# lfilipozzi/PathPlanning

Hardware: AMD Instinct MI355X
Metric: hybrid_astar_plans_per_sec_1024x1024 (higher is better)
Workload: dtype f64

## Files before the change

__graft_entry__.py:

```python
import os
import subprocess
import sys

os.environ.setdefault("GPU_MAX_HW_QUEUES", "2")

ROOT = os.path.dirname(os.path.abspath(__file__))
if ROOT not in sys.path:
    sys.path.insert(0, ROOT)


def build():
    from pathplanning_amd import build as b
    lib = b.build(force=False)
    assert os.path.exists(lib), lib
    b.build_pyplanning()
    b.build_plugin_test()
    b.build_pipeline_footprint_test()
    b.build_pipeline_postprocess_test()
    b.build_pipeline_revalidate_test()
    b.build_pipeline_stamp_test()
    b.build_stamp_rule_test()
    b.build_ticket_table_test()
    b.build_row_test()
    subprocess.check_call(["make", "-C", os.path.join(ROOT, "oracle"), os.path.join(ROOT, "oracle", "libppo.so")])
    if os.path.isdir("/root/reference/planner/src"):
        subprocess.check_call(["make", "-C", os.path.join(ROOT, "oracle"), "ref"])
    subprocess.check_call([sys.executable, "-c", "import ctypes, sys; ctypes.CDLL(sys.argv[1])", lib])
    import pathplanning_amd
    print("built", lib)


def smoke():
    sys.path.insert(0, os.path.join(ROOT, "tests"))
    import numpy as np
    import pathplanning_amd as pa
    import torch
    assert torch.cuda.is_available(), "smoke() needs a GPU"
    import oracle_lib as O
    w = O.synthetic_world(256, 6, 3)
    ctx = pa.Context(0)
    ms = pa.OccupancyMapSet.from_bounds(ctx, w.lb, w.ub, 0.1)
    ms.upload_dist2(w.d2())
    ms.upload_occupancy(w.occ())
    ms.upload_path_cost(w.pathcost())
    val = pa.StateValidatorOccupancyMap(ms)
    rng = np.random.RandomState(0)
    poses = np.column_stack([rng.uniform(-13, 13, 4096), rng.uniform(-13, 13, 4096), rng.uniform(-3.1, 3.1, 4096)])
    got = val.is_state_valid(poses)
    want = w.is_state_valid(poses).astype(bool)
    assert np.array_equal(got, want), "check_states mismatch"
    planner = pa.HybridAStarBatch(val, max_batch=2, max_nodes=32768)
    planner.initialize()
    starts = [[-10.0, -10.0, 0.0], [9.0, -9.0, 1.0]]
    goals = [[10.0, 10.0, 0.0], [-9.0, 8.0, -2.0]]
    res = planner.search_batch(starts, goals, [7, 8])
    h = O.Hybrid(w, table=planner.nonholo_table())
    for q in range(2):
        r = h.search(starts[q], goals[q], 7 + q)
        assert res[q].status == r["status"], (res[q].status, r["status"])
        assert np.array_equal(planner.get_expanded_of(q), r["expanded"]), "expansion order mismatch"
        if r["status"] == 0:
            assert abs(res[q].cost - r["cost"]) < 1e-5
    sys.path.insert(0, os.path.join(ROOT, "tests"))
    from gpu_common import valid_random_poses
    n = 72
    big = pa.HybridAStarBatch(val, max_batch=n, max_nodes=32768, search_rows=16)
    big.initialize()
    bs, bg = valid_random_poses(rng, w, n), valid_random_poses(rng, w, n)
    seeds = np.arange(n, dtype=np.uint64) + 100
    bres = big.search_batch(bs, bg, seeds)
    for q in range(0, n, 6):
        r = h.search(bs[q], bg[q], int(seeds[q]))
        assert bres[q].status == r["status"] and bres[q].n_expanded == len(r["expanded"]), (q, bres[q].status, bres[q].n_expanded, r["status"], len(r["expanded"]))
        assert np.array_equal(big.get_expanded_of(q), r["expanded"]), "expansion order mismatch (rows kernel)"
    import time
# ... 35 lines not shown
```

pathplanning_amd/build.py:

```python
import os
import subprocess
import sys

HERE = os.path.dirname(os.path.abspath(__file__))
CSRC = os.path.join(HERE, "csrc")
LIB_DIR = os.path.join(HERE, "lib")
LIB = os.path.join(LIB_DIR, "libpphip.so")
SOURCES = ["pp_capi.hip", "pp_kernels_basic.hip", "pp_paths.hip", "pp_footprint.hip", "pp_gvd.hip", "pp_wavefront.hip", "pp_wavefront_tiles.hip", "pp_planner.hip", "pp_rrt.hip", "pp_grid_astar.hip"]
HEADERS = sorted(f for f in os.listdir(CSRC) if f.endswith(".hpp")) + [os.path.join("..", "..", "include", "pp_hip.h")]
FLAGS = ["--offload-arch=gfx950", "-O3", "-std=c++17", "-ffp-contract=off", "-fPIC", "-shared"]


def hipcc():
    for c in (os.environ.get("HIPCC"), "/opt/rocm/bin/hipcc", "hipcc"):
        if c and (os.path.isabs(c) and os.path.exists(c) or not os.path.isabs(c)):
            return c
    return "hipcc"


def stale():
    if not os.path.exists(LIB):
        return True
    t = os.path.getmtime(LIB)
    deps = [os.path.join(CSRC, s) for s in SOURCES + HEADERS]
# ... 48 lines not shown
    cmd = ["g++", "-O2", "-std=c++17", src, "-o", out, "-L" + LIB_DIR, "-lpphip", "-Wl,-rpath,$ORIGIN"]
    if verbose:
        print(" ".join(cmd), file=sys.stderr)
    subprocess.check_call(cmd)
    return out


def build_pipeline_postprocess_test(verbose=True):
    build()
    out = os.path.join(LIB_DIR, "test_pipeline_postprocess")
    src = os.path.join(HERE, "..", "tests", "cpp", "test_pipeline_postprocess.cpp")
    cmd = ["g++", "-O2", "-std=c++17", src, "-o", out, "-L" + LIB_DIR, "-lpphip", "-Wl,-rpath,$ORIGIN"]
    if verbose:
        print(" ".join(cmd), file=sys.stderr)
    subprocess.check_call(cmd)
    return out


def build_pipeline_revalidate_test(verbose=True):
    build()
    out = os.path.join(LIB_DIR, "test_pipeline_revalidate")
    src = os.path.join(HERE, "..", "tests", "cpp", "test_pipeline_revalidate.cpp")
    cmd = ["g++", "-O2", "-std=c++17", src, "-o", out, "-L" + LIB_DIR, "-lpphip", "-Wl,-rpath,$ORIGIN"]
    if verbose:
        print(" ".join(cmd), file=sys.stderr)
    subprocess.check_call(cmd)
    return out


def build_pipeline_stamp_test(verbose=True):
    build()
    out = os.path.join(LIB_DIR, "test_pipeline_stamp")
    src = os.path.join(HERE, "..", "tests", "cpp", "test_pipeline_stamp.cpp")
    cmd = ["g++", "-O2", "-std=c++17", src, "-o", out, "-L" + LIB_DIR, "-lpphip", "-Wl,-rpath,$ORIGIN"]
    if verbose:
        print(" ".join(cmd), file=sys.stderr)
    subprocess.check_call(cmd)
    return out


def build_stamp_rule_test(verbose=True):
    os.makedirs(LIB_DIR, exist_ok=True)
    out = os.path.join(LIB_DIR, "test_stamp_rule")
    src = os.path.join(HERE, "..", "tests", "cpp", "test_stamp_rule.cpp")
    if os.path.exists(out) and os.path.getmtime(out) > max(os.path.getmtime(src), os.path.getmtime(os.path.join(CSRC, "pp_stamp_rule.hpp"))):
        return out
    cmd = ["g++", "-std=c++17", "-g", "-O1", "-ffp-contract=off", "-fsanitize=address,undefined", "-fno-sanitize-recover=all", "-I", CSRC, src, "-o", out]
    if verbose:
        print(" ".join(cmd), file=sys.stderr)
    subprocess.check_call(cmd)
    return out


def build_ticket_table_test(verbose=True):
    os.makedirs(LIB_DIR, exist_ok=True)
    out = os.path.join(LIB_DIR, "test_ticket_table")
    src = os.path.join(HERE, "..", "tests", "cpp", "test_ticket_table.cpp")
    if os.path.exists(out) and os.path.getmtime(out) > max(os.path.getmtime(src), os.path.getmtime(os.path.join(CSRC, "pp_ticket_table.hpp"))):
        return out
    cmd = ["g++", "-std=c++17", "-g", "-fsanitize=address,undefined", "-fno-sanitize-recover=all", "-I", CSRC, src, "-o", out]
    if verbose:
        print(" ".join(cmd), file=sys.stderr)
    subprocess.check_call(cmd)
    return out


def build_row_test(verbose=True):
    out = os.path.join(LIB_DIR, "test_row_primitives")
    src = os.path.join(HERE, "..", "tests", "cpp", "test_row_primitives.hip")
    if os.path.exists(out) and os.path.getmtime(out) > max(os.path.getmtime(src), os.path.getmtime(os.path.join(CSRC, "pp_row_primitives.hpp"))):
        return out
    cmd = [hipcc(), "--offload-arch=gfx950", "-O2", "-I", CSRC, "-I", os.path.join(HERE, "..", "include"), src, "-o", out]
    if verbose:
        print(" ".join(cmd), file=sys.stderr)
    subprocess.check_call(cmd)
    return out


if __name__ == "__main__":
    build(force="--force" in sys.argv)
    print(LIB)
    print(build_pyplanning())
    print(build_plugin_test())
    print(build_pipeline_footprint_test())
    print(build_pipeline_postprocess_test())
    print(build_pipeline_revalidate_test())
    print(build_pipeline_stamp_test())
    print(build_stamp_rule_test())
    print(build_ticket_table_test())
    print(build_row_test())
```

pathplanning_amd/csrc/pp_planner.hip:

```cpp
#include "pp_search_device.hpp"
#include "pp_row_primitives.hpp"
#include "pp_stamp_rule.hpp"

#include <cmath>
#include <cstring>
#include <memory>
#include <string>
#include <utility>
#include <vector>

using namespace ppd;

namespace {

struct Node {
	double x, y, t;
	double pathCost, totalCost;
	double length;
	double h;
	double sinT, cosT;
	int32_t parent;
	uint32_t key;
	int16_t action;
	uint8_t dead;
	uint8_t pad0;
	float dist0;
	uint8_t pad[8];
};
static_assert(sizeof(Node) == 96, "Node layout");

struct PathRec {
	double x, y, t, length;
	int32_t action;
	int32_t node;
};
static_assert(sizeof(PathRec) == 40, "PathRec layout");

struct SuspendRec {
	int32_t q, slot;
	int32_t heapSize, nNodes, nExpanded, nRngDraws, nRsAttempts, nRsLog, mtIdx;
	uint32_t seq;
	long long stateChecks, pathChecks;
	long long bandLo;
	int32_t nOutside, pad;
};

struct RsLogEntry {
	int32_t node, word;
	double t, u, v;
};
constexpr int kRsLogCap = 64;

struct KeySpace {
	int x0, y0, t0;
// ... 424 lines not shown
		if (a.from != a.from || a.to != a.to) {
			set_error(what(i) + " has a NaN in its window");
			return PP_ERR_INVALID;
		}
	}
	return PP_OK;
}

Footprint stamp_discs(const pp_footprint* fp, const pp_map* own)
{
	if (fp)
		return fp->fp;
	Footprint f {};
	f.n = 1;
	f.r[0] = own->minSafeRadius;
	return f;
}

int stamp_prepare_target(pp_map* map)
{
	if (map->occ32)
		return PP_OK;
	const size_t n = map->cells();
	PP_HIP_TRY(map->occ32.ensure(n * 4));
	PP_HIP_TRY(hipMemsetAsync(map->occ32, 0xFF, n * 4, map->ctx->stream));
	PP_HIP_TRY(hipStreamSynchronize(map->ctx->stream));
	return PP_OK;
}

int stamp_finish_target(pp_map* map)
{
	map->journal.clear();
	map->journal.shrink_to_fit();
	map->journalLost = true;
	if (int rc = pph::refresh_occupancy_views(map, map->ctx->stream))
		return rc;
	PP_HIP_TRY(hipStreamSynchronize(map->ctx->stream));
	return PP_OK;
}

template <typename Rec>
void records_out(const std::vector<Rec>& host, Rec* out)
{
	if (out)
		std::copy(host.begin(), host.end(), out);
}

void free_planner(pp_planner* p)
{
	if (!p)
		return;
#if PP_ROWS_STATS
	{
		unsigned long long h[24] = {};
		if (hipMemcpyFromSymbol(h, HIP_SYMBOL(g_rowsStats), sizeof h) == hipSuccess) {
			fprintf(stderr, "[rows stats] wave iterations with 1/2/3/4 busy rows: %llu %llu %llu %llu\n", h[1], h[2], h[3], h[4]);
			static const char* const names[14] = { "take", "set-aside", "pop+refill", "node", "child validity", "march", "truncate+cost", "cell-node+staging", "insert", "write", "rs", "endpoint", "keymap+heuristics", "voronoi" };
			unsigned long long tot = 0, it = h[1] + h[2] + h[3] + h[4];
			for (int i = 0; i < 14; i++)
				tot += h[8 + i];
			for (int i = 0; i < 14; i++)
				fprintf(stderr, "[rows stats]   %-18s %5.1f %%  %8.0f clk / wave iteration\n", names[i], 100.0 * (double)h[8 + i] / (double)(tot ? tot : 1), (double)h[8 + i] / (double)(it ? it : 1));
		}
	}
#endif
	pp_map* map = p->map;
	pph::footprint_release(p->footprint);
	delete p;
	pph::map_release(map);
}

}

enum class PlannerUse { Batches, Pipeline, PipelineLogged };
static int create_planner(pp_map* map, const pp_hybrid_params* params, int32_t max_batch, int32_t max_nodes_per_query, int32_t search_rows, PlannerUse use, pp_planner** out);

extern "C" {

int pp_planner_create(pp_map* map, const pp_hybrid_params* params, int32_t max_batch, int32_t max_nodes_per_query, pp_planner** out)
{
	return pp_planner_create_ex(map, params, max_batch, max_nodes_per_query, 0, out);
}

int pp_planner_create_ex(pp_map* map, const pp_hybrid_params* params, int32_t max_batch, int32_t max_nodes_per_query, int32_t search_rows, pp_planner** out)
{
	return create_planner(map, params, max_batch, max_nodes_per_query, search_rows, PlannerUse::Batches, out);
}

static int create_planner(pp_map* map, const pp_hybrid_params* params, int32_t max_batch, int32_t max_nodes_per_query, int32_t search_rows, PlannerUse use, pp_planner** out)
{
	const bool forPipeline = use != PlannerUse::Batches;
	if (!map || !params || !out || max_batch < 1 || max_nodes_per_query < 16 || search_rows < 0) {
		set_error("invalid arguments");
		return PP_ERR_INVALID;
	}
	if (!map->dist || !map->occ8 || !map->pathcost) {
		set_error("map set incomplete: upload dist2, occupancy and path cost first");
		return PP_ERR_INVALID;
	}
	PP_HIP_TRY(hipSetDevice(map->ctx->device));
	auto* p = new pp_planner();
	p->map = map;
	__atomic_add_fetch(&map->refs, 1, __ATOMIC_RELAXED);
	p->params = *params;
	p->maxBatch = max_batch;
	p->maxNodes = max_nodes_per_query;

	const double wheelbase = params->wheelbase, rearToCenter = 0.0;
	const double deltaMax = std::atan(wheelbase / std::sqrt(std::pow(params->min_turning_radius, 2) - std::pow(rearToCenter, 2)));
	p->deltas.push_back(0.0);
	for (unsigned int i = 0; i < params->num_generated_motion / 2; i++) {
		double delta = (i + 1) / 2.0 * deltaMax;
		p->deltas.push_back(delta);
		p->deltas.push_back(-delta);
	}
// ... 893 lines not shown
```

pathplanning_amd/csrc/pp_planner_rows.hpp:

```cpp
#ifndef PP_ROWS_FOOTPRINT
#error "pp_planner_rows.hpp is the body of the rows kernels of pp_planner.hip, which defines PP_ROWS_FOOTPRINT before each include"
#endif

#ifndef PP_ROWS_PREAMBLE_DONE
#define PP_ROWS_PREAMBLE_DONE 1
#ifndef PP_ROWS_STATS
#define PP_ROWS_STATS 0
#endif
#if PP_ROWS_STATS
__device__ unsigned long long g_rowsStats[24];
#endif
#ifndef PP_ROWS_WAVES_PER_WG
#define PP_ROWS_WAVES_PER_WG 4
#endif
#if PP_ROWS_STATS
#undef PP_ROWS_WAVES_PER_WG
#define PP_ROWS_WAVES_PER_WG 1
#endif
#ifndef PP_ROWS_EAGER_REFILL
#define PP_ROWS_EAGER_REFILL 1
#endif

#ifndef PP_PIPE_POLL_EVERY
#define PP_PIPE_POLL_EVERY 8
#endif
constexpr int kPollEvery = PP_PIPE_POLL_EVERY;
#endif

#if PP_ROWS_FOOTPRINT
#define PP_ROWS_KERNEL k_hybrid_search_rows_footprint
#define PP_ROWS_FOOT_ARG Footprint foot,
#else
#define PP_ROWS_KERNEL k_hybrid_search_rows
#define PP_ROWS_FOOT_ARG
#endif
template <bool kPiped>
__global__ void __launch_bounds__(64 * PP_ROWS_WAVES_PER_WG, PP_SEARCH_WAVES_PER_SIMD) PP_ROWS_KERNEL(SearchArgs A, PP_ROWS_FOOT_ARG int nQueries, const double* __restrict__ starts,
	const double* __restrict__ goals, const uint64_t* __restrict__ seeds, const float* __restrict__ costFields, Node* __restrict__ nodesBase,
	HeapEntry* __restrict__ heapBase, uint32_t* __restrict__ keymapBase, uint32_t* __restrict__ expandedBase, RsLogEntry* __restrict__ rsLogBase,
	PathRec* __restrict__ pathBase, unsigned long long* __restrict__ mtBase, DevResult* __restrict__ results, int* __restrict__ nextQuery,
	SuspendRec* __restrict__ suspended, const int32_t* __restrict__ order, int suspendAfter, int* __restrict__ suspendedCount, int* __restrict__ spareCount,
	HeapEntry* __restrict__ bandBase, double bandInvW, uint8_t* __restrict__ bandMetaBase, PipeView pipe)
{
#if PP_SEARCH_SETPRIO
	__builtin_amdgcn_s_setprio(PP_ROWS_PRIO);
#endif
	constexpr int kW = kPiped ? 1 : PP_ROWS_WAVES_PER_WG;
	const int lane = threadIdx.x & 63;
	const int waveIdx = (int)blockIdx.x * kW + (int)(threadIdx.x >> 6);
	if (waveIdx >= A.rowsWaves)
		return;
	const int rl = lane & (kRowLanes - 1);
	const int sb = (lane >> 4) * kRowSlots;
	constexpr bool piped = kPiped;
	if (piped) {
		int owner = 0;
		if (lane == 0)
			owner = __hip_atomic_compare_exchange_strong(pipe.waveAlive + waveIdx, &owner, 1, __ATOMIC_RELAXED, __ATOMIC_RELAXED, __HIP_MEMORY_SCOPE_AGENT) ? 0 : 1;
		if (__builtin_amdgcn_readfirstlane(owner))
			return;
		__builtin_amdgcn_fence(__ATOMIC_ACQUIRE, "agent");
	}
	int idleIters = 0;
// ... 52 lines not shown
	long long laneStateChecks = 0, lanePathChecks = 0, rsStateChecks = 0, rsPathChecks = 0;

	auto flush_spills = [&]() {
		wave_lds_sync();
		bool toHeap = false;
		if (rl < nSpill) {
			const HeapEntry mine = spillBuf[rl];
			const long long B = band_of_key(mine.ckey, bandInvW);
			toHeap = true;
			if (B >= bandLo && B < bandLo + kBands) {
				const int sl = (int)(B & (kBands - 1)), sh = (sl & 3) * 8;
				const uint32_t old = atomicAdd(&bandCnt[sl >> 2], 1u << sh);
				const int pos = (int)((old >> sh) & 0xFFu);
				if (pos < kBandCap) {
					ROW_BANDS[sl * kBandCap + pos] = mine;
					toHeap = false;
				} else {
					atomicSub(&bandCnt[sl >> 2], 1u << sh);
				}
			}
		}
		uint32_t hm = row_bits(__ballot(toHeap), lane);
		if (__builtin_expect(hm != 0u, false)) {
			wave_vmem_sync();
			if (rl == 0) {
				int hs = heapSize;
				for (uint32_t mm = hm; mm; mm &= mm - 1)
					heap_push(ROW_HEAP, hs, spillBuf[__ffs((int)mm) - 1]);
			}
			for (; hm; hm &= hm - 1) {
				const HeapEntry e = spillBuf[__ffs((int)hm) - 1];
				if (heapSize == 0 || heap_before(e, heapTop))
					heapTop = e;
				heapSize++;
			}
		}
		nSpill = 0;
		wave_lds_sync();
		wave_vmem_sync();
	};
	auto spill = [&](const HeapEntry& e) {
		if (!bandLoSet) {
			bandLo = (band_of_key(e.ckey, bandInvW) - 64) & ~3ll;
			bandLoSet = true;
		}
		if (rl == 0)
			spillBuf[nSpill] = e;
		nSpill++;
		nOutside++;
		if (key_before(e.ckey, e.nseq, lowK, lowS)) {
			lowK = e.ckey;
			lowS = e.nseq;
		}
		if (nSpill == kRowLanes)
			flush_spills();
	};
	auto push_open = [&](const HeapEntry& e) {
		bool toFront = true;
		if (frontCount < kRowLanes)
			toFront = nOutside == 0 || key_before(e.ckey, e.nseq, lowK, lowS) ||
				(frontCount > 0 && key_before(e.ckey, e.nseq, row_read64(front.ckey, lane, frontCount - 1), row_read(front.nseq, lane, frontCount - 1)));
		if (toFront) {
			HeapEntry sp;
			if (front_insert_row(front, frontCount, e, rl, lane, sp))
				spill(sp);
		} else {
			spill(e);
		}
	};
	auto refill = [&]() {
		if (nSpill > 0)
			flush_spills();
		long long bAbs = 0x7FFFFFFFFFFFFFFFll;
		const int w0 = (int)(bandLo >> 2);
#pragma unroll 1
		for (int step = 0; step < kBands / 64; step++) {
			const uint32_t w = bandCnt[(w0 + step * kRowLanes + rl) & (kBands / 4 - 1)];
			const uint32_t hit = row_bits(__ballot(w != 0u), lane);
			if (hit) {
				const int fl = __ffs((int)hit) - 1;
				const uint32_t wf = row_read(w, lane, fl);
				bAbs = bandLo + 4ll * (step * kRowLanes + fl) + ((__ffs((int)wf) - 1) >> 3);
				break;
			}
		}
		long long loadedTop = bandLo - 1;
		if (bAbs != 0x7FFFFFFFFFFFFFFFll) {
			const int sl = (int)(bAbs & (kBands - 1)), sh = (sl & 3) * 8;
			const int n = (int)((bandCnt[sl >> 2] >> sh) & 0xFFu);
			HeapEntry e;
			e.ckey = ~0ull;
			e.nseq = ~0u;
			e.node = 0;
			if (rl < n)
				e = ROW_BANDS[sl * kBandCap + rl];
			row_sort_entries(e.ckey, e.nseq, e.node, rl);
			front.ckey = e.ckey;
			front.nseq = e.nseq;
			front.node = e.node;
			frontCount = n;
			nOutside -= n;
			wave_lds_sync();
			if (rl == 0)
				bandCnt[sl >> 2] &= ~(0xFFu << sh);
			wave_lds_sync();
			bandLo = bAbs & ~3ll;
			loadedTop = bAbs;
		}
		lowK = ~0ull;
		lowS = ~0u;
		while (__builtin_expect(heapSize > 0 && (frontCount == 0 || key_before(heapTop.ckey, heapTop.nseq, row_read64(front.ckey, lane, frontCount - 1), row_read(front.nseq, lane, frontCount - 1))), false)) {
			wave_vmem_sync();
			const HeapEntry he = heap_pop_row(ROW_HEAP, heapSize, rl, lane, heapTop);
			wave_vmem_sync();
			nOutside--;
			HeapEntry sp;
			if (front_insert_row(front, frontCount, he, rl, lane, sp))
				spill(sp);
		}
		if (heapSize > 0 && key_before(heapTop.ckey, heapTop.nseq, lowK, lowS)) {
			lowK = heapTop.ckey;
			lowS = heapTop.nseq;
		}
		{
			const unsigned long long bk = cost_key((double)(loadedTop + 1) / bandInvW);
			if (bk < lowK || (bk == lowK && 0u < lowS)) {
				lowK = bk;
				lowS = 0u;
			}
		}
		wave_lds_sync();
		for (int i = 0; i < nSpill; i++) {
			const HeapEntry e = spillBuf[i];
			if (key_before(e.ckey, e.nseq, lowK, lowS)) {
				lowK = e.ckey;
				lowS = e.nseq;
			}
		}
	};
	auto set_slot = [&](size_t sl_) {
		slot = (int)sl_;
		nodes = nodesBase + (size_t)slot * A.maxNodes;
		keymap = keymapBase + (size_t)slot * A.ks.size();
	};
	auto finish = [&](const int status, const int solutionNode, const double solutionCost) {
		const long long nStateChecks = row_sum_i64(laneStateChecks, lane) + rsStateChecks;
		const long long pathChecksPacked = row_sum_i64(lanePathChecks, lane) + rsPathChecks;
		const long long pathChecks = pathChecksPacked & kGuardMask;
		wave_vmem_sync();
		if (rl == 0) {
			DevResult r;
			r.r.n_lattice_boundary_hits = (int32_t)(pathChecksPacked >> kGuardShift);
			r.r.reserved = 0;
			r.r.status = status;
			r.r.n_expanded = nExpanded;
			r.r.n_nodes = nNodes;
			r.r.n_path = 0;
			if (status == 0)
				r.r.n_path = write_path(nodes, solutionNode, pathBase + (size_t)q * A.maxPath, A.maxPath, piped ? pipe.pathHost + (size_t)q * (size_t)(3 * pipe.pathHostCap) : nullptr,
					piped ? pipe.pathHostCap : 0);
			r.r.cost = solutionCost;
			r.r.n_rng_draws = nRngDraws;
			r.r.n_rs_attempts = nRsAttempts;
			r.r.n_state_checks = nStateChecks;
			r.r.n_path_checks = pathChecks;
			r.solutionNode = solutionNode;
			r.nRsLog = nRsLog < kRsLogCap ? nRsLog : kRsLogCap;
			results[q] = r;
			if (piped) {
				__builtin_amdgcn_fence(__ATOMIC_RELEASE, "");
				asm volatile("s_waitcnt vmcnt(0)" ::: "memory");
				const unsigned long long d = __hip_atomic_fetch_add(&pipe.ctl->doneTail, 1ull, __ATOMIC_RELAXED, __HIP_MEMORY_SCOPE_AGENT);
				PipeDone* const rec = pipe.done + (d & pipe.doneMask);
				rec->r = r;
				rec->readyTail = __hip_atomic_load(&pipe.ctl->readyTail, __ATOMIC_RELAXED, __HIP_MEMORY_SCOPE_AGENT);
				rec->readyHead = __hip_atomic_load(&pipe.ctl->readyHead, __ATOMIC_RELAXED, __HIP_MEMORY_SCOPE_AGENT);
				__builtin_amdgcn_fence(__ATOMIC_RELEASE, "");
				asm volatile("s_waitcnt vmcnt(0)" ::: "memory");
				__hip_atomic_store(&rec->stamp, ((d + 1ull) << 32) | (unsigned long long)(uint32_t)q, __ATOMIC_RELAXED, __HIP_MEMORY_SCOPE_SYSTEM);
			}
		}
		act = false;
		pollNow = true;
	};

#if PP_ROWS_STATS
	unsigned long long statIter[5] = { 0, 0, 0, 0, 0 };
	__shared__ unsigned long long s_phase[16], s_tlast;
	if (lane < 16)
		s_phase[lane] = 0ull;
	if (lane == 0)
		s_tlast = clock64();
	wave_lds_sync();
#define ROWS_STAMP(ph)                                                     \
	{                                                                      \
		const unsigned long long now_ = clock64();                        \
		if (lane == __ffsll((long long)__ballot(true)) - 1) {             \
			s_phase[ph] += now_ - s_tlast;                                \
			s_tlast = now_;                                               \
		}                                                                  \
	}
#else
#define ROWS_STAMP(ph)
#endif
	int endStatus, endNode;
	double endCost;
	for (;;) {
		if (false) {
		row_query_ends:
			finish(endStatus, endNode, endCost);
		}
		if (__builtin_expect(!act && !done, false)) {
			bool none = false;
			if (piped) {
				int got = -1;
				const bool look = pollNow || (passCount % (unsigned)kPollEvery) == 0u;
				if (rl == 0 && look) {
					unsigned long long h = __hip_atomic_load(&pipe.ctl->readyHead, __ATOMIC_RELAXED, __HIP_MEMORY_SCOPE_AGENT);
					const unsigned long long e = __hip_atomic_load(pipe.ready + (h & pipe.readyMask), __ATOMIC_RELAXED, __HIP_MEMORY_SCOPE_AGENT);
					if ((uint32_t)(e >> 32) == (uint32_t)(h + 1ull))
						got = __hip_atomic_compare_exchange_strong(&pipe.ctl->readyHead, &h, h + 1ull, __ATOMIC_RELAXED, __ATOMIC_RELAXED, __HIP_MEMORY_SCOPE_AGENT)
							? (int)(uint32_t)e : -2;
				}
				q = (int)row_read((uint32_t)got, lane, 0);
				none = q < 0;
				pollNow = q == -2;
				if (!none) {
					__builtin_amdgcn_fence(__ATOMIC_ACQUIRE, "agent");
				}
			} else {
				int nq = 0;
				if (rl == 0)
					nq = atomicAdd(nextQuery, 1);
				q = (int)row_read((uint32_t)nq, lane, 0);
				if (q >= nQueries) {
					done = true;
					none = true;
				}
			}
			if (!none) {
				if (order)
					q = order[q];
				field = costFields + (size_t)q * A.fieldElems;
				const RowsClaim claim = rows_claim_init<PP_ROWS_FOOTPRINT != 0>(q, field, nodes, keymap, ROW_MT, bandCnt, starts, goals, seeds, rows_kernarg_segment());
				goal = { claim.gx, claim.gy, claim.gt };
				myNode = -1;
				rsNode = -1;
				pfNode = -1;
				pfDead = false;
				noSuspend = false;
				front_clear(front);
				frontCount = 0;
				heapSize = 0;
				nSpill = 0;
				nOutside = 0;
				bandLo = 0;
// ... 313 lines not shown
				const Node* fn = nodes + (st - 1u);
				fpx = fn->x;
				fpy = fn->y;
				fpt = fn->t;
				fptot = fn->totalCost;
				fpFor = st;
			}
			if (base == 0) {
				int cand = -1;
				if (frontCount > 0)
					cand = (int)row_read(front.node, lane, 0);
				pfNode = cand;
				pfDead = false;
				if (cand >= 0 && rl < 11)
					pf64 = reinterpret_cast<const unsigned long long*>(nodes + cand)[rl];
			}
			const bool dup = row_earlier_same(key, ok, rl);
			c_key[sb + rl] = key;
			c_state[sb + rl] = st;
			c_flags[sb + rl] = (uint8_t)((ok ? 1 : 0) | (dup ? 2 : 0));
			c_x[sb + rl] = child.x;
			c_y[sb + rl] = child.y;
			c_t[sb + rl] = child.t;
			c_cost[sb + rl] = gcost;
			c_total[sb + rl] = total;
			c_len[sb + rl] = len;
			c_h[sb + rl] = hh;
			c_sin[sb + rl] = cs;
			c_cos[sb + rl] = cc;
			c_d0[sb + rl] = d0;
			f_x[sb + rl] = fpx;
			f_y[sb + rl] = fpy;
			f_t[sb + rl] = fpt;
			f_tot[sb + rl] = fptot;
			f_for[sb + rl] = fpFor;
			myNode = -1;
			wave_lds_sync();
			ROWS_STAMP(7)
			const int cnt = min(kRowLanes, P - base);
			bool need = false;
			if (rl < cnt && ok) {
				if (dup || st == 0u)
					need = true;
				else if (st != kExplored) {
					if (fpFor == st) {
						const Pose fpp = { fpx, fpy, fpt };
						need = identical_poses(fpp, child) && fptot > total;
					} else {
						need = true;
					}
				}
			}
			uint32_t todo = row_bits(__ballot(need), lane);
			while (todo != 0u) {
				const int c = __ffs((int)todo) - 1;
				todo &= todo - 1u;
				const uint32_t flags = c_flags[sb + c];
				if (!(flags & 1u) || capacity)
					continue;
				const uint32_t ckey = c_key[sb + c];
				uint32_t cst = c_state[sb + c];
				if (flags & 2u) {
					wave_vmem_sync();
					cst = keymap[ckey];
				}
				const double ctotal = c_total[sb + c];
				bool push = false;
				if (cst == 0u) {
					push = true;
				} else if (cst != kExplored) {
					const int fi = (int)cst - 1;
					const uint32_t hitf = row_bits(__ballot(myNode == fi), lane);
					Pose fp;
					double ftotal;
					if (hitf) {
						const int fs = __ffs((int)hitf) - 1;
						fp = { c_x[sb + fs], c_y[sb + fs], c_t[sb + fs] };
						ftotal = c_total[sb + fs];
					} else if (f_for[sb + c] == cst) {
						fp = { f_x[sb + c], f_y[sb + c], f_t[sb + c] };
						ftotal = f_tot[sb + c];
					} else {
						wave_vmem_sync();
						const Node fn = nodes[fi];
						fp = { fn.x, fn.y, fn.t };
						ftotal = fn.totalCost;
					}
					const Pose cp = { c_x[sb + c], c_y[sb + c], c_t[sb + c] };
					if (identical_poses(fp, cp) && ftotal > ctotal) {
						if (fi == pfNode)
							pfDead = true;
						if (rl == 0)
							nodes[fi].dead = 1;
						if (myNode == fi)
							myNode = -1;
						push = true;
					}
				}
				if (push) {
					if (nNodes >= maxNodes) {
						capacity = true;
						continue;
					}
					const int idx = nNodes++;
					if (rl == c)
						myNode = idx;
					if (rl == 0)
						keymap[ckey] = (uint32_t)idx + 1u;
					HeapEntry e;
					e.ckey = cost_key(ctotal);
					e.nseq = 0xFFFFFFFFu - seq;
					seq++;
					e.node = (uint32_t)idx;
					push_open(e);
				}
			}
			ROWS_STAMP(8)
			if (myNode >= 0) {
				Node nd;
				nd.x = child.x;
				nd.y = child.y;
				nd.t = child.t;
				nd.pathCost = gcost;
				nd.totalCost = total;
				nd.length = len;
				nd.h = hh;
				nd.sinT = cs;
				nd.cosT = cc;
				nd.parent = ni;
				nd.key = key;
				nd.action = (int16_t)p;
				nd.dead = 0;
				nd.dist0 = d0;
				nodes[myNode] = nd;
			}
		}
		ROWS_STAMP(9)
		if (__builtin_expect(capacity, false)) {
			endStatus = -4, endNode = -1, endCost = __builtin_huge_val();
			goto row_query_ends;
		}

		bool tryRs = !gateDraws;
		if (gateDraws) {
			if (mtIdx >= Mt64::N) {
				wave_vmem_sync();
				mt_twist_row(ROW_MT, rl);
				mtIdx = 0;
				mtRaw = ROW_MT[0];
			}
			const double u = Mt64::uniform01(Mt64::temper(mtRaw));
			mtIdx++;
			nRngDraws++;
			tryRs = u < 10.0 / (hCost * hCost);
		}
		if (__builtin_expect(tryRs, false)) {
			nRsAttempts++;
			const RowsRsResult rsr = rows_rs_attempt<PP_ROWS_FOOTPRINT != 0>(px, py, pt, pSin, pCos, goal.x, goal.y, goal.t, pPathCost, field, keymap, &W, rows_kernarg_segment());
			const int word = rsr.word;
			if (word >= 0) {
				const double bt = rsr.t, bu = rsr.u, bv = rsr.v;
				lanePathChecks += (long long)rsr.boundary << kGuardShift;
				rsPathChecks++;
				rsStateChecks += (long long)rsr.checks;
				if (rsr.valid) {
					const uint32_t ckey = c_key[sb + kRowRs];
					const uint32_t cst = c_state[sb + kRowRs];
					bool push = false;
					if (cst == 0u)
// ... 16 lines not shown
						const Pose cp = { c_x[sb + kRowRs], c_y[sb + kRowRs], c_t[sb + kRowRs] };
						if (identical_poses(fp, cp) && ftotal > c_total[sb + kRowRs]) {
							if (fi == pfNode)
								pfDead = true;
							if (rl == 0)
								nodes[fi].dead = 1;
							if (myNode == fi)
								myNode = -1;
							push = true;
						}
					}
					if (push) {
						if (nNodes >= maxNodes) {
							endStatus = -4, endNode = -1, endCost = __builtin_huge_val();
							goto row_query_ends;
						}
						const int idx = nNodes++;
						if (rl == 0) {
							Node nd;
							nd.x = c_x[sb + kRowRs];
							nd.y = c_y[sb + kRowRs];
							nd.t = c_t[sb + kRowRs];
							nd.pathCost = c_cost[sb + kRowRs];
							nd.totalCost = c_total[sb + kRowRs];
							nd.length = c_len[sb + kRowRs];
							nd.h = c_h[sb + kRowRs];
							nd.sinT = c_sin[sb + kRowRs];
							nd.cosT = c_cos[sb + kRowRs];
							nd.parent = ni;
							nd.key = ckey;
							nd.action = c_action[sb + kRowRs];
							nd.dead = 0;
							nd.dist0 = c_d0[sb + kRowRs];
							nodes[idx] = nd;
							keymap[ckey] = (uint32_t)idx + 1u;
							if (nRsLog < kRsLogCap) {
								RsLogEntry le;
								le.node = idx;
								le.word = word;
								le.t = bt;
								le.u = bu;
								le.v = bv;
								(rsLogBase + (size_t)q * kRsLogCap)[nRsLog] = le;
							}
						}
						rsNode = idx;
						nRsLog++;
						HeapEntry e;
						e.ckey = cost_key(c_total[sb + kRowRs]);
						e.nseq = 0xFFFFFFFFu - seq;
						seq++;
						e.node = (uint32_t)idx;
						push_open(e);
					}
				}
				wave_lds_sync();
			}
		}
		ROWS_STAMP(10)
	}
#if PP_ROWS_STATS
	if (lane == 0)
		for (int i = 1; i < 5; i++)
			atomicAdd(&g_rowsStats[i], statIter[i]);
	wave_lds_sync();
	if (lane < 14)
		atomicAdd(&g_rowsStats[8 + lane], s_phase[lane]);
#endif
#undef ROWS_STAMP
#undef ROW_HEAP
#undef ROW_MT
#undef ROW_BANDS
}
#undef PP_ROWS_KERNEL
#undef PP_ROWS_FOOT_ARG
```

pathplanning_amd/csrc/pp_row_primitives.hpp:

```cpp
#pragma once
#include "pp_search_device.hpp"

namespace ppd {

PPD_INLINE void row_vmem_sync()
{
	__builtin_amdgcn_fence(__ATOMIC_ACQ_REL, "workgroup");
	__builtin_amdgcn_s_waitcnt(0);
	__builtin_amdgcn_wave_barrier();
}

constexpr int kRowLanes = 16;
constexpr int kRowsPerWave = 4;
constexpr int kRowSlots = kRowLanes + 1;
constexpr int kRowRs = kRowLanes;

PPD_INLINE uint32_t row_bits(unsigned long long ballot, int lane) { return (uint32_t)(ballot >> (lane & 48)) & 0xFFFFu; }
PPD_INLINE uint32_t row_read(uint32_t v, int lane, int c) { return (uint32_t)__builtin_amdgcn_ds_bpermute(((lane & 48) | c) << 2, (int)v); }
PPD_INLINE unsigned long long row_read64(unsigned long long v, int lane, int c)
{
	return ((unsigned long long)row_read((uint32_t)(v >> 32), lane, c) << 32) | row_read((uint32_t)v, lane, c);
}
PPD_INLINE double row_read_f64(double v, int lane, int c) { return __longlong_as_double((long long)row_read64((unsigned long long)__double_as_longlong(v), lane, c)); }
PPD_INLINE uint32_t row_shr1(uint32_t v, uint32_t fill) { return (uint32_t)__builtin_amdgcn_update_dpp((int)fill, (int)v, 0x111, 0xF, 0xF, false); }
PPD_INLINE uint32_t row_shl1(uint32_t v, uint32_t fill) { return (uint32_t)__builtin_amdgcn_update_dpp((int)fill, (int)v, 0x101, 0xF, 0xF, false); }
PPD_INLINE unsigned long long row_shr1_64(unsigned long long v, unsigned long long fill)
{
	return ((unsigned long long)row_shr1((uint32_t)(v >> 32), (uint32_t)(fill >> 32)) << 32) | row_shr1((uint32_t)v, (uint32_t)fill);
}
PPD_INLINE unsigned long long row_shl1_64(unsigned long long v, unsigned long long fill)
{
	return ((unsigned long long)row_shl1((uint32_t)(v >> 32), (uint32_t)(fill >> 32)) << 32) | row_shl1((uint32_t)v, (uint32_t)fill);
}
PPD_INLINE uint32_t row_min_u32(uint32_t v)
{
	uint32_t x = v;
	x = min(x, (uint32_t)__builtin_amdgcn_update_dpp((int)x, (int)x, 0xB1, 0xF, 0xF, false));
	x = min(x, (uint32_t)__builtin_amdgcn_update_dpp((int)x, (int)x, 0x4E, 0xF, 0xF, false));
	x = min(x, (uint32_t)__builtin_amdgcn_update_dpp((int)x, (int)x, 0x141, 0xF, 0xF, false));
	x = min(x, (uint32_t)__builtin_amdgcn_update_dpp((int)x, (int)x, 0x140, 0xF, 0xF, false));
	return x;
}
PPD_INLINE long long row_sum_i64(long long v, int lane)
{
	long long x = v;
#pragma unroll
	for (int off = 8; off > 0; off >>= 1)
		x += __shfl_xor(x, off, 64);
	return x;
}
PPD_INLINE int row_argmin_key(unsigned long long k, uint32_t s, int lane, unsigned long long& mk, uint32_t& ms)
{
	const uint32_t hi = (uint32_t)(k >> 32), lo = (uint32_t)k;
	const uint32_t mhi = row_min_u32(hi);
	bool cand = hi == mhi;
	const uint32_t mlo = row_min_u32(cand ? lo : 0xFFFFFFFFu);
	cand = cand && lo == mlo;
	ms = row_min_u32(cand ? s : 0xFFFFFFFFu);
	cand = cand && s == ms;
	mk = ((unsigned long long)mhi << 32) | mlo;
	return __ffs((int)row_bits(__ballot(cand), lane)) - 1;
}
PPD_INLINE bool row_earlier_same(uint32_t key, bool flag, int rl)
{
	const uint32_t f = flag ? 1u : 0u;
	bool dup = false;
#define PP_ROR(n)                                                                                                    \
	{                                                                                                                \
		const uint32_t k_ = (uint32_t)__builtin_amdgcn_update_dpp(0, (int)key, 0x120 + (n), 0xF, 0xF, false);         \
		const uint32_t f_ = (uint32_t)__builtin_amdgcn_update_dpp(0, (int)f, 0x120 + (n), 0xF, 0xF, false);           \
		dup = dup || ((n) <= rl && f_ != 0u && k_ == key);        \
	}
	PP_ROR(1) PP_ROR(2) PP_ROR(3) PP_ROR(4) PP_ROR(5) PP_ROR(6) PP_ROR(7) PP_ROR(8) PP_ROR(9) PP_ROR(10) PP_ROR(11) PP_ROR(12) PP_ROR(13) PP_ROR(14) PP_ROR(15)
#undef PP_ROR
	return dup;
}

PPD_INLINE bool front_insert_row(FrontLane& f, int& count, const HeapEntry& e, int rl, int lane, HeapEntry& spilled)
{
	const bool mineFirst = rl < count && key_before(f.ckey, f.nseq, e.ckey, e.nseq);
	const int pos = __popc(row_bits(__ballot(mineFirst), lane));
	if (pos >= kRowLanes) {
		spilled = e;
		return true;
	}
	bool spill = false;
	if (count == kRowLanes) {
		spilled.ckey = row_read64(f.ckey, lane, kRowLanes - 1);
		spilled.nseq = row_read(f.nseq, lane, kRowLanes - 1);
		spilled.node = row_read(f.node, lane, kRowLanes - 1);
		spill = true;
	}
	const unsigned long long uk = row_shr1_64(f.ckey, ~0ull);
	const uint32_t us = row_shr1(f.nseq, ~0u);
	const uint32_t un = row_shr1(f.node, 0u);
	if (rl > pos) {
		f.ckey = uk;
		f.nseq = us;
		f.node = un;
	} else if (rl == pos) {
		f.ckey = e.ckey;
		f.nseq = e.nseq;
// ... 132 lines not shown
```

pathplanning_amd/csrc/pp_rows_rs.hpp:

```cpp
#pragma once

struct RowsWaveLds {
	static constexpr int kS = kRowsPerWave * kRowSlots;
	double c_x[kS], c_y[kS], c_t[kS], c_cost[kS], c_total[kS], c_len[kS], c_h[kS], c_sin[kS], c_cos[kS];
	double f_x[kS], f_y[kS], f_t[kS], f_tot[kS];
	HeapEntry spill[kRowsPerWave][kRowLanes];
	uint32_t bandCnt[kRowsPerWave][kBands / 4];
	uint32_t c_key[kS], c_state[kS], f_for[kS];
	float c_d0[kS];
	int rsChecks[kRowsPerWave];
	double rsPre[kRowsPerWave][24];
	int16_t c_action[kS];
	uint8_t c_flags[kS], c_valid[kS];
};
static_assert(offsetof(RowsWaveLds, bandCnt) % 16 == 0 && sizeof(RowsWaveLds) % 16 == 0, "band counters are copied as uint4");

struct RowsKernargHead {
	SearchArgs A;
	Footprint foot;
};
__device__ __forceinline__ uint64_t rows_kernarg_segment()
{
	return (uint64_t)(uintptr_t)__builtin_amdgcn_kernarg_segment_ptr();
}
__device__ __forceinline__ const RowsKernargHead& rows_kernargs(const uint64_t segment)
{
	typedef const __attribute__((address_space(4))) RowsKernargHead* SegPtr;
	const uint32_t lo = __builtin_amdgcn_readfirstlane((uint32_t)segment), hi = __builtin_amdgcn_readfirstlane((uint32_t)(segment >> 32));
	return *(const RowsKernargHead*)(SegPtr)(uintptr_t)(((uint64_t)hi << 32) | lo);
}

struct SinCosPair {
	double s, c;
};
__device__ __attribute__((noinline)) SinCosPair rows_arc_sincos(const double t)
{
	SinCosPair r;
	sincos(t, &r.s, &r.c);
	return r;
}
struct SinCosShared {
	PPD_INLINE static void eval(double t, double& s, double& c)
	{
		const SinCosPair r = rows_arc_sincos(t);
		s = r.s;
		c = r.c;
	}
};
using RowsArc = ArcSCT<SinCosShared>;

#define PP_ROWS_MATH1(name) \
	__device__ __attribute__((noinline)) double rows_##name(const double x) { return ::name(x); }
PP_ROWS_MATH1(sin)
PP_ROWS_MATH1(cos)
PP_ROWS_MATH1(acos)
PP_ROWS_MATH1(asin)
#undef PP_ROWS_MATH1
__device__ __attribute__((noinline)) double rows_atan2(const double y, const double x) { return ::atan2(y, x); }
__device__ __attribute__((noinline)) double rows_fmod(const double x, const double y) { return ::fmod(x, y); }
// ... 226 lines not shown
```

Before: 38480.

## Batch-insert plain children into spill buffer in one pass during expansion

Adds a fast path to child insertion: when every child needing insertion is a plain new cell that sorts outside the front's bound, all are assigned node ids and written to the spill buffer at once by rank, replacing the serial per-child walk. The spill buffer is doubled so a batch can overflow, with a flush loop draining it. The spill lower bound is now a row-wide min reduction instead of a serial scan. Also adds stats counters and a host unit test for the batch rule. Risks: extra shuffles and LDS use, plus subtle ordering issues in the open list.

```diff
diff --git a/__graft_entry__.py b/__graft_entry__.py
--- a/__graft_entry__.py
+++ b/__graft_entry__.py
@@ -21,6 +21,7 @@
     b.build_pipeline_stamp_test()
     b.build_stamp_rule_test()
     b.build_ticket_table_test()
+    b.build_open_batch_rule_test()
     b.build_row_test()
     subprocess.check_call(["make", "-C", os.path.join(ROOT, "oracle"), os.path.join(ROOT, "oracle", "libppo.so")])
     if os.path.isdir("/root/reference/planner/src"):
diff --git a/pathplanning_amd/build.py b/pathplanning_amd/build.py
--- a/pathplanning_amd/build.py
+++ b/pathplanning_amd/build.py
@@ -124,6 +124,19 @@
     return out
 
 
+def build_open_batch_rule_test(verbose=True):
+    os.makedirs(LIB_DIR, exist_ok=True)
+    out = os.path.join(LIB_DIR, "test_open_batch_rule")
+    src = os.path.join(HERE, "..", "tests", "cpp", "test_open_batch_rule.cpp")
+    if os.path.exists(out) and os.path.getmtime(out) > max(os.path.getmtime(src), os.path.getmtime(os.path.join(CSRC, "pp_open_batch_rule.hpp"))):
+        return out
+    cmd = ["g++", "-std=c++17", "-g", "-O1", "-fsanitize=address,undefined", "-fno-sanitize-recover=all", "-I", CSRC, src, "-o", out]
+    if verbose:
+        print(" ".join(cmd), file=sys.stderr)
+    subprocess.check_call(cmd)
+    return out
+
+
 def build_ticket_table_test(verbose=True):
     os.makedirs(LIB_DIR, exist_ok=True)
     out = os.path.join(LIB_DIR, "test_ticket_table")
diff --git a/pathplanning_amd/csrc/pp_open_batch_rule.hpp b/pathplanning_amd/csrc/pp_open_batch_rule.hpp
--- /dev/null
+++ b/pathplanning_amd/csrc/pp_open_batch_rule.hpp
@@ -0,0 +1,24 @@
+#pragma once
+#include <cstdint>
+
+#if defined(__HIPCC__)
+#define PPOB_INLINE __host__ __device__ __forceinline__
+#else
+#define PPOB_INLINE inline
+#endif
+
+namespace ppob {
+
+PPOB_INLINE bool before(unsigned long long ak, unsigned int as, unsigned long long bk, unsigned int bs) { return ak < bk || (ak == bk && as < bs); }
+
+PPOB_INLINE bool plain_child(unsigned int cellState, bool earlierChildSharesCell) { return cellState == 0u && !earlierChildSharesCell; }
+
+PPOB_INLINE bool outside_bound(int frontCount, int frontCap, int nOutside, unsigned long long ek, unsigned int es, unsigned long long lowK, unsigned int lowS,
+	unsigned long long lastK, unsigned int lastS)
+{
+	if (frontCount >= frontCap)
+		return !before(ek, es, lastK, lastS);
+	return nOutside > 0 && !before(ek, es, lowK, lowS) && !(frontCount > 0 && before(ek, es, lastK, lastS));
+}
+
+}
diff --git a/pathplanning_amd/csrc/pp_planner.hip b/pathplanning_amd/csrc/pp_planner.hip
--- a/pathplanning_amd/csrc/pp_planner.hip
+++ b/pathplanning_amd/csrc/pp_planner.hip
@@ -1,5 +1,6 @@
 #include "pp_search_device.hpp"
 #include "pp_row_primitives.hpp"
+#include "pp_open_batch_rule.hpp"
 #include "pp_stamp_rule.hpp"
 
 #include <cmath>
@@ -530,7 +531,7 @@
 		return;
 #if PP_ROWS_STATS
 	{
-		unsigned long long h[24] = {};
+		unsigned long long h[40] = {};
 		if (hipMemcpyFromSymbol(h, HIP_SYMBOL(g_rowsStats), sizeof h) == hipSuccess) {
 			fprintf(stderr, "[rows stats] wave iterations with 1/2/3/4 busy rows: %llu %llu %llu %llu\n", h[1], h[2], h[3], h[4]);
 			static const char* const names[14] = { "take", "set-aside", "pop+refill", "node", "child validity", "march", "truncate+cost", "cell-node+staging", "insert", "write", "rs", "endpoint", "keymap+heuristics", "voronoi" };
@@ -539,6 +540,15 @@
 				tot += h[8 + i];
 			for (int i = 0; i < 14; i++)
 				fprintf(stderr, "[rows stats]   %-18s %5.1f %%  %8.0f clk / wave iteration\n", names[i], 100.0 * (double)h[8 + i] / (double)(tot ? tot : 1), (double)h[8 + i] / (double)(it ? it : 1));
+			unsigned long long ins = 0, passes = 0;
+			for (int i = 0; i <= 10; i++)
+				ins += h[24 + i], passes += (unsigned long long)i * h[24 + i];
+			fprintf(stderr, "[rows stats] insertion: wave iterations by passes of the walk, 0..10+:");
+			for (int i = 0; i <= 10; i++)
+				fprintf(stderr, " %.1f %%", 100.0 * (double)h[24 + i] / (double)(ins ? ins : 1));
+			fprintf(stderr, "  (mean %.2f)\n", (double)passes / (double)(ins ? ins : 1));
+			fprintf(stderr, "[rows stats] insertion: rows with a batch to push: %llu in one pass, %llu walked (%.1f %% in one pass)\n", h[35], h[36],
+				100.0 * (double)h[35] / (double)(h[35] + h[36] ? h[35] + h[36] : 1));
 		}
 	}
 #endif
diff --git a/pathplanning_amd/csrc/pp_planner_rows.hpp b/pathplanning_amd/csrc/pp_planner_rows.hpp
--- a/pathplanning_amd/csrc/pp_planner_rows.hpp
+++ b/pathplanning_amd/csrc/pp_planner_rows.hpp
@@ -8,7 +8,7 @@
 #define PP_ROWS_STATS 0
 #endif
 #if PP_ROWS_STATS
-__device__ unsigned long long g_rowsStats[24];
+__device__ unsigned long long g_rowsStats[40];
 #endif
 #ifndef PP_ROWS_WAVES_PER_WG
 #define PP_ROWS_WAVES_PER_WG 4
@@ -167,8 +167,15 @@
 			lowK = e.ckey;
 			lowS = e.nseq;
 		}
-		if (nSpill == kRowLanes)
-			flush_spills();
+	};
+	auto lower_bound_to = [&](const unsigned long long k, const uint32_t s) {
+		unsigned long long mk;
+		uint32_t ms;
+		row_min_key(k, s, mk, ms);
+		if (key_before(mk, ms, lowK, lowS)) {
+			lowK = mk;
+			lowS = ms;
+		}
 	};
 	auto push_open = [&](const HeapEntry& e) {
 		bool toFront = true;
@@ -230,8 +237,11 @@
 			wave_vmem_sync();
 			nOutside--;
 			HeapEntry sp;
-			if (front_insert_row(front, frontCount, he, rl, lane, sp))
+			if (front_insert_row(front, frontCount, he, rl, lane, sp)) {
 				spill(sp);
+				if (nSpill == kRowLanes)
+					flush_spills();
+			}
 		}
 		if (heapSize > 0 && key_before(heapTop.ckey, heapTop.nseq, lowK, lowS)) {
 			lowK = heapTop.ckey;
@@ -245,12 +255,14 @@
 			}
 		}
 		wave_lds_sync();
-		for (int i = 0; i < nSpill; i++) {
-			const HeapEntry e = spillBuf[i];
-			if (key_before(e.ckey, e.nseq, lowK, lowS)) {
-				lowK = e.ckey;
-				lowS = e.nseq;
-			}
+		{
+			unsigned long long sk = ~0ull;
+			uint32_t ss = ~0u;
+			if (rl < nSpill) {
+				sk = spillBuf[rl].ckey;
+				ss = spillBuf[rl].nseq;
+			}
+			lower_bound_to(sk, ss);
 		}
 	};
 	auto set_slot = [&](size_t sl_) {
@@ -301,9 +313,9 @@
 
 #if PP_ROWS_STATS
 	unsigned long long statIter[5] = { 0, 0, 0, 0, 0 };
-	__shared__ unsigned long long s_phase[16], s_tlast;
+	__shared__ unsigned long long s_phase[16], s_tlast, s_ins[16];
 	if (lane < 16)
-		s_phase[lane] = 0ull;
+		s_phase[lane] = s_ins[lane] = 0ull;
 	if (lane == 0)
 		s_tlast = clock64();
 	wave_lds_sync();
@@ -315,8 +327,22 @@
 			s_tlast = now_;                                               \
 		}                                                                  \
 	}
+#define ROWS_COUNT(i, by)                                  \
+	if (lane == __ffsll((long long)__ballot(true)) - 1)    \
+		s_ins[i] += (unsigned long long)(by);
+#define ROWS_COUNT_ROW(i) \
+	if (rl == 0)          \
+		atomicAdd(&s_ins[i], 1ull);
+#define ROWS_PASSES_DONE()                                                     \
+	if (lane == __ffsll((long long)__ballot(true)) - 1) {                      \
+		s_ins[s_ins[13] < 10ull ? s_ins[13] : 10ull]++;                        \
+		s_ins[13] = 0ull;                                                      \
+	}
 #else
 #define ROWS_STAMP(ph)
+#define ROWS_COUNT(i, by)
+#define ROWS_COUNT_ROW(i)
+#define ROWS_PASSES_DONE()
 #endif
 	int endStatus, endNode;
 	double endCost;
@@ -736,7 +762,52 @@
 				}
 			}
 			uint32_t todo = row_bits(__ballot(need), lane);
-			while (todo != 0u) {
+			{
+				const int n = __popc(todo);
+				int rlHere = rl;
+				asm volatile("" : "+v"(rlHere));
+				const int rank = __popc(todo & ((1u << rlHere) - 1u));
+				HeapEntry me;
+				me.ckey = cost_key(total);
+				me.nseq = 0xFFFFFFFFu - (seq + (uint32_t)rank);
+				const int lastI = (frontCount - 1) & (kRowLanes - 1);
+				const unsigned long long lastK = row_read64(front.ckey, lane, lastI);
+				const uint32_t lastS = row_read(front.nseq, lane, lastI);
+				const bool fits = !need || (ppob::plain_child(st, dup) && ppob::outside_bound(frontCount, kRowLanes, nOutside, me.ckey, me.nseq, lowK, lowS, lastK, lastS));
+				if (todo != 0u && row_bits(__ballot(!fits), lane) == 0u && nNodes + n <= maxNodes) {
+					ROWS_COUNT_ROW(11)
+					if (!bandLoSet) {
+						bandLo = (band_of_key(row_read64(me.ckey, lane, __ffs((int)todo) - 1), bandInvW) - 64) & ~3ll;
+						bandLoSet = true;
+					}
+					if (need) {
+						myNode = nNodes + rank;
+						keymap[key] = (uint32_t)myNode + 1u;
+						me.node = (uint32_t)myNode;
+						spillBuf[nSpill + rank] = me;
+					}
+					lower_bound_to(need ? me.ckey : ~0ull, need ? me.nseq : ~0u);
+					nSpill += n;
+					nOutside += n;
+					nNodes += n;
+					seq += (uint32_t)n;
+					todo = 0u;
+				} else if (todo != 0u) {
+					ROWS_COUNT_ROW(12)
+				}
+			}
+			while (todo != 0u || nSpill >= kRowLanes) {
+				if (nSpill >= kRowLanes) {
+					const int rest = nSpill - kRowLanes;
+					nSpill = kRowLanes;
+					flush_spills();
+					if (rl < rest)
+						spillBuf[rl] = spillBuf[kRowLanes + rl];
+					nSpill = rest;
+					wave_lds_sync();
+					continue;
+				}
+				ROWS_COUNT(13, 1)
 				const int c = __ffs((int)todo) - 1;
 				todo &= todo - 1u;
 				const uint32_t flags = c_flags[sb + c];
@@ -799,6 +870,7 @@
 					push_open(e);
 				}
 			}
+			ROWS_PASSES_DONE()
 			ROWS_STAMP(8)
 			if (myNode >= 0) {
 				Node nd;
@@ -921,6 +993,8 @@
 						seq++;
 						e.node = (uint32_t)idx;
 						push_open(e);
+						if (nSpill == kRowLanes)
+							flush_spills();
 					}
 				}
 				wave_lds_sync();
@@ -935,8 +1009,13 @@
 	wave_lds_sync();
 	if (lane < 14)
 		atomicAdd(&g_rowsStats[8 + lane], s_phase[lane]);
+	if (lane < 13)
+		atomicAdd(&g_rowsStats[24 + lane], s_ins[lane]);
 #endif
 #undef ROWS_STAMP
+#undef ROWS_COUNT
+#undef ROWS_COUNT_ROW
+#undef ROWS_PASSES_DONE
 #undef ROW_HEAP
 #undef ROW_MT
 #undef ROW_BANDS
diff --git a/pathplanning_amd/csrc/pp_row_primitives.hpp b/pathplanning_amd/csrc/pp_row_primitives.hpp
--- a/pathplanning_amd/csrc/pp_row_primitives.hpp
+++ b/pathplanning_amd/csrc/pp_row_primitives.hpp
@@ -48,6 +48,14 @@
 	for (int off = 8; off > 0; off >>= 1)
 		x += __shfl_xor(x, off, 64);
 	return x;
+}
+PPD_INLINE void row_min_key(unsigned long long k, uint32_t s, unsigned long long& mk, uint32_t& ms)
+{
+	const uint32_t hi = (uint32_t)(k >> 32), lo = (uint32_t)k;
+	const uint32_t mhi = row_min_u32(hi);
+	const uint32_t mlo = row_min_u32(hi == mhi ? lo : 0xFFFFFFFFu);
+	ms = row_min_u32(hi == mhi && lo == mlo ? s : 0xFFFFFFFFu);
+	mk = ((unsigned long long)mhi << 32) | mlo;
 }
 PPD_INLINE int row_argmin_key(unsigned long long k, uint32_t s, int lane, unsigned long long& mk, uint32_t& ms)
 {
diff --git a/pathplanning_amd/csrc/pp_rows_rs.hpp b/pathplanning_amd/csrc/pp_rows_rs.hpp
--- a/pathplanning_amd/csrc/pp_rows_rs.hpp
+++ b/pathplanning_amd/csrc/pp_rows_rs.hpp
@@ -4,7 +4,7 @@
 	static constexpr int kS = kRowsPerWave * kRowSlots;
 	double c_x[kS], c_y[kS], c_t[kS], c_cost[kS], c_total[kS], c_len[kS], c_h[kS], c_sin[kS], c_cos[kS];
 	double f_x[kS], f_y[kS], f_t[kS], f_tot[kS];
-	HeapEntry spill[kRowsPerWave][kRowLanes];
+	HeapEntry spill[kRowsPerWave][2 * kRowLanes];
 	uint32_t bandCnt[kRowsPerWave][kBands / 4];
 	uint32_t c_key[kS], c_state[kS], f_for[kS];
 	float c_d0[kS];
```

Measured after the change: 29600. 0.769x the previous value.
